# Yixin-F/DR-Using-SCV-OD

Measured on AMD Instinct MI355X. Metric: scans/sec on SemanticKITTI-seq-05-shaped input (SCV-OD dynamic-removal path, raw scans -> per-point labels + static map), higher is better.
Workload: dtype f32

## Files before the change

dr-using-scv-od_amd/csrc/scvod_k_patchwork.inc:

```
constexpr int kClsThreads = 256;
constexpr int kClsItems = 8;

__global__ __launch_bounds__(kClsThreads) void k_pw_classify(DevParams P, Arena A) {
    __shared__ int hist[kMaxPatches];
    const int s = blockIdx.y;
    const int base = A.scan_off[s];
    const int n = A.scan_off[s + 1] - base;
    const int start = blockIdx.x * (kClsThreads * kClsItems);
    if (start >= n) return;
    for (int b = threadIdx.x; b < P.n_patches; b += kClsThreads) hist[b] = 0;
    __syncthreads();
    float4 pt[kClsItems];
#pragma unroll
    for (int it = 0; it < kClsItems; ++it) {
        const int i = start + it * kClsThreads + threadIdx.x;
        pt[it] = A.pts[base + min(i, n - 1)];
    }
#pragma unroll
    for (int it = 0; it < kClsItems; ++it) {
        const int i = start + it * kClsThreads + threadIdx.x;
        if (i < n) {
            const float4 p = pt[it];
            int pid = czm_patch_of(P.czm, p.x, p.y, p.z);
            A.pid[base + i] = (int16_t)pid;
            A.zkey[base + i] = float_sort_key(p.z);
            if (pid >= 0) atomicAdd(&hist[pid], 1);
        }
    }
    __syncthreads();
    for (int b = threadIdx.x; b < P.n_patches; b += kClsThreads) {
        int c = hist[b];
        if (c) atomicAdd(&A.patch_count[s * kMaxPatches + b], c);
    }
}

__global__ __launch_bounds__(1024) void k_pw_offsets(DevParams P, Arena A) {
    __shared__ int wsum[17];
    const int s = blockIdx.x;
    int c = (threadIdx.x < (unsigned)P.n_patches) ? A.patch_count[s * kMaxPatches + threadIdx.x] : 0;
    int total;
    int ex = block_excl_scan<1024>(c, total, wsum);
    if (threadIdx.x <= (unsigned)P.n_patches) A.patch_off[s * (kMaxPatches + 1) + threadIdx.x] = ex;
}

__global__ __launch_bounds__(kClsThreads) void k_pw_scatter(DevParams P, Arena A) {
    __shared__ int hist[kMaxPatches];
    const int s = blockIdx.y;
    const int base = A.scan_off[s];
    const int n = A.scan_off[s + 1] - base;
    const int start = blockIdx.x * (kClsThreads * kClsItems);
    if (start >= n) return;
    for (int b = threadIdx.x; b < P.n_patches; b += kClsThreads) hist[b] = 0;
    __syncthreads();
    int pid[kClsItems], rank[kClsItems];
    uint32_t zk[kClsItems];
#pragma unroll
    for (int it = 0; it < kClsItems; ++it) {
        const int i = start + it * kClsThreads + threadIdx.x;
        pid[it] = (i < n) ? (int)A.pid[base + i] : -1;
        zk[it] = A.zkey[base + min(i, n - 1)];
    }
#pragma unroll
    for (int it = 0; it < kClsItems; ++it)
        rank[it] = wave_bin_rank(hist, pid[it]);
    __syncthreads();
    for (int b = threadIdx.x; b < P.n_patches; b += kClsThreads) {
        int c = hist[b];
        if (c) hist[b] = A.patch_off[s * (kMaxPatches + 1) + b] + atomicAdd(&A.patch_cursor[s * kMaxPatches + b], c);
    }
    __syncthreads();
#pragma unroll
    for (int it = 0; it < kClsItems; ++it) {
        int i = start + it * kClsThreads + threadIdx.x;
        if (i < n && pid[it] >= 0) A.keys[(size_t)base + hist[pid[it]] + rank[it]] = pack_key(zk[it], (uint32_t)i);
    }
}

constexpr int kClassXS = 32, kClassM = 40, kClassM2 = 44, kClassL = 48;
#ifndef SCVOD_FIT_COOP_CLASS
#define SCVOD_FIT_COOP_CLASS 36
#endif
constexpr int kClassFitCoop = SCVOD_FIT_COOP_CLASS;

__device__ __forceinline__ void order_range(const int32_t* off, int c_lo, int c_hi, int& lo, int& hi) {
    lo = off[c_hi];
    hi = (c_lo == 0) ? off[64] : off[c_lo - 1];
}

constexpr bool pw_sort_padfree(int cap) { return SCVOD_SORT_PADFREE == 2 || (SCVOD_SORT_PADFREE == 1 && cap >= 2048); }
constexpr bool pw_sort_merge(int cap) {
    return pw_sort_padfree(cap) && cap >= 2048 && cap <= 8192 && (SCVOD_SORT_MERGE == 2 || (SCVOD_SORT_MERGE == 1 && cap >= 4096));
}

template <int CAP, int THREADS, int C_LO, int C_HI, int LGE>
__global__ __launch_bounds__(THREADS)
__attribute__((amdgpu_waves_per_eu(pw_sort_padfree(CAP) ? (CAP >= 1024 ? 4 : 6) : 1, 8)))
void k_pw_sort(DevParams P, Arena A) {
    extern __shared__ __attribute__((aligned(16))) unsigned char smem[];
    int lo, hi;
    order_range(A.order_off, C_LO, C_HI, lo, hi);
    constexpr int PK = (CAP == 4096) ? 1 : 2;
    constexpr bool PADFREE = pw_sort_padfree(CAP);
    constexpr bool MERGE = pw_sort_merge(CAP) && LGE == 4 && (THREADS << LGE) == CAP;
    PROF_BEGIN();
    for (int w = lo + blockIdx.x; w < hi; w += gridDim.x) {
        const int4 item = A.order[w];
        const int n = item.y, base = item.z, off = item.w;
        const bool in_lds = (n <= CAP);
        unsigned long long* keys;
        if (CAP >= 4096) PROF_RESET();
        if (in_lds) {
            keys = (unsigned long long*)smem;
            int np2 = 1 << LGE;
            while (np2 < n) np2 <<= 1;
            const int nlive = sortnet::live_end(n, LGE);
            constexpr int IT = CAP / THREADS;
            const unsigned long long* gk = (const unsigned long long*)A.keys + (size_t)base + off;
            bool from_regs = false;
            if constexpr (IT == (1 << LGE) && CAP >= 4096) {
                if (np2 == CAP) {
                    from_regs = true;
                    unsigned long long tmp[IT];
                    if constexpr (PADFREE) {
                        if ((int)threadIdx.x < (nlive >> LGE)) {
#pragma unroll
                            for (int it = 0; it < IT; ++it) {
                                const int j = sortnet::start_key(it, (int)threadIdx.x, nlive, LGE);
                                tmp[it] = (j < n) ? gk[j] : kKeyPad;
                            }
                        }
                        if (CAP >= 4096) PROF_MARK(PK, 0);
                        if constexpr (MERGE)
                            mergepath_sort_regs<THREADS, true, LGE, SCVOD_SORT_MERGE_RUN>(tmp, keys, np2, nlive, (unsigned long long)kKeyPad);
                        else
                            padfree_sort_regs<THREADS, true, LGE>(tmp, keys, np2, nlive, (unsigned long long)kKeyPad);
                    } else {
#pragma unroll
                        for (int it = 0; it < IT; ++it) {
                            const int j = it * THREADS + (int)threadIdx.x;
                            tmp[it] = (j < n) ? gk[j] : kKeyPad;
                        }
                        if (CAP >= 4096) PROF_MARK(PK, 0);
                        block_bitonic_sort_pow2_regs<THREADS, true, LGE>(tmp, keys);
                    }
                }
            }
            if (!from_regs) {
                const int nfill = PADFREE ? nlive : np2;
                for (int j = threadIdx.x; j < nfill; j += THREADS) keys[sort_slot<true>(j)] = (j < n) ? gk[j] : kKeyPad;
                __syncthreads();
                if (CAP >= 4096) PROF_MARK(PK, 0);
                if constexpr (MERGE)
                    mergepath_sort<THREADS, true, LGE, SCVOD_SORT_MERGE_RUN>(keys, np2, nlive, (unsigned long long)kKeyPad);
                else if constexpr (PADFREE)
                    padfree_sort<THREADS, true, LGE>(keys, np2, nlive, (unsigned long long)kKeyPad);
                else
                    block_bitonic_sort_pow2<THREADS, true, LGE>(keys, np2);
            }
            if (CAP >= 4096) PROF_MARK(PK, 1);
        } else {
            keys = (unsigned long long*)(A.keys + (size_t)base + off);
            block_bitonic_sort<THREADS, false>(keys, n);
        }
        Xyz* dst = A.sorted_xyz + (size_t)base + off;
        uint32_t* dsti = A.sorted_idx + (size_t)base + off;
        for (int j0 = threadIdx.x; j0 < n; j0 += 4 * THREADS) {
            uint32_t id[4];
            float4 q[4];
#pragma unroll
            for (int u = 0; u < 4; ++u) {
                const int j = min(j0 + u * THREADS, n - 1);
                id[u] = key_idx(keys[in_lds ? sort_slot<true>(j) : j]);
            }
#pragma unroll
            for (int u = 0; u < 4; ++u) q[u] = A.pts[base + id[u]];
#pragma unroll
            for (int u = 0; u < 4; ++u) {
                const int j = j0 + u * THREADS;
                if (j < n) {
                    Xyz o;
                    o.x = q[u].x;
                    o.y = q[u].y;
                    o.z = q[u].z;
                    dst[j] = o;
                    dsti[j] = id[u];
                }
            }
        }
        __syncthreads();
        if (CAP >= 4096) PROF_MARK(PK, 2);
    }
}

constexpr int kClassWave = 24;
__global__ __launch_bounds__(256) void k_pw_sort_wave(DevParams P, Arena A) {
    const int lane = threadIdx.x & 63;
    const int wave = threadIdx.x >> 6;
    int lo, hi;
    order_range(A.order_off, 0, kClassWave - 1, lo, hi);
    for (int w = lo + blockIdx.x * 4 + wave; w < hi; w += gridDim.x * 4) {
        const int4 item = A.order[w];
        const int n = item.y, base = item.z, off = item.w;
        unsigned long long key = (lane < n) ? A.keys[(size_t)base + off + lane] : kKeyPad;
#pragma unroll
        for (int k = 2; k <= 64; k <<= 1) {
#pragma unroll
            for (int j = k >> 1; j >= 1; j >>= 1) {
                const unsigned long long other = __shfl_xor(key, j, 64);
                const bool take_min = (((lane & k) == 0) == ((lane & j) == 0));
                unsigned long long mn = key, mx = other;
                cswap_asc(mn, mx);
                key = take_min ? mn : mx;
            }
        }
        if (lane < n) {
            const uint32_t id = key_idx(key);
            const float4 q = A.pts[base + id];
            Xyz o;
            o.x = q.x;
            o.y = q.y;
            o.z = q.z;
            A.sorted_xyz[(size_t)base + off + lane] = o;
            A.sorted_idx[(size_t)base + off + lane] = id;
        }
    }
}

__device__ __forceinline__ int pw_size_class(int n) {
    int lg = 31 - __clz(n);
    int frac = (lg >= 2) ? ((n >> (lg - 2)) & 3) : 0;
    int c = lg * 4 + frac;
    return c > 63 ? 63 : c;
}

__global__ __launch_bounds__(256) void k_pw_order_count(DevParams P, Arena A) {
    __shared__ int hist[64];
    if (threadIdx.x < 64) hist[threadIdx.x] = 0;
    __syncthreads();
    const int t = blockIdx.x * 256 + threadIdx.x;
    if (t < A.n_scans * P.n_patches) {
        const int s = t / P.n_patches, p = t - s * P.n_patches;
        const int n = A.patch_count[s * kMaxPatches + p];
        if (n <= P.czm.num_min_pts) {
            PatchRec r = {n, 0, 0, 0, 0};
            A.patch_rec[s * kMaxPatches + p] = r;
            scvod_patch_plane pl = {};
            pl.n_pts = n;
            A.planes[s * kMaxPatches + p] = pl;
        } else {
            atomicAdd(&hist[pw_size_class(n)], 1);
        }
    }
    __syncthreads();
    if (threadIdx.x < 64 && hist[threadIdx.x]) atomicAdd(&A.order_hist[threadIdx.x], hist[threadIdx.x]);
}

__global__ __launch_bounds__(64) void k_pw_order_offsets(Arena A) {
    const int c = 63 - threadIdx.x;
    const int v = A.order_hist[c];
    const int inc = wave_incl_scan(v);
    A.order_off[c] = inc - v;
    if (threadIdx.x == 63) A.order_off[64] = inc;
}

__global__ __launch_bounds__(256) void k_pw_order_scatter(DevParams P, Arena A) {
    __shared__ int hist[64];
    if (threadIdx.x < 64) hist[threadIdx.x] = 0;
    __syncthreads();
    const int t = blockIdx.x * 256 + threadIdx.x;
    int c = -1, rank = 0;
    int4 item = make_int4(0, 0, 0, 0);
    if (t < A.n_scans * P.n_patches) {
        const int s = t / P.n_patches, p = t - s * P.n_patches;
        const int n = A.patch_count[s * kMaxPatches + p];
        if (n > P.czm.num_min_pts) {
            c = pw_size_class(n);
            rank = atomicAdd(&hist[c], 1);
            item = make_int4(s * kMaxPatches + p, n, A.scan_off[s], A.patch_off[s * (kMaxPatches + 1) + p]);
        }
    }
    __syncthreads();
    if (threadIdx.x < 64 && hist[threadIdx.x])
        hist[threadIdx.x] = A.order_off[threadIdx.x] + atomicAdd(&A.order_cursor[threadIdx.x], hist[threadIdx.x]);
    __syncthreads();
    if (c >= 0) A.order[hist[c] + rank] = item;
}

__global__ __launch_bounds__(256) void k_vx_order_count(DevParams P, Arena A) {
    __shared__ int hist[64];
    if (threadIdx.x < 64) hist[threadIdx.x] = 0;
    __syncthreads();
    const int t = blockIdx.x * 256 + threadIdx.x;
    if (t < A.n_scans * P.n_buckets) {
        const int s = t / P.n_buckets, b = t - s * P.n_buckets;
        const int m = A.vb_count[s * kMaxBuckets + b];
        if (m > 0)
            atomicAdd(&hist[pw_size_class(m)], 1);
        else
            A.vb_nvox[s * kMaxBuckets + b] = 0;
    }
    __syncthreads();
    if (threadIdx.x < 64 && hist[threadIdx.x]) atomicAdd(&A.vorder_hist[threadIdx.x], hist[threadIdx.x]);
}

__global__ __launch_bounds__(64) void k_vx_order_offsets(Arena A) {
    const int c = 63 - threadIdx.x;
    const int v = A.vorder_hist[c];
    const int inc = wave_incl_scan(v);
    A.vorder_off[c] = inc - v;
    if (threadIdx.x == 63) A.vorder_off[64] = inc;
}

__global__ __launch_bounds__(256) void k_vx_order_scatter(DevParams P, Arena A) {
    __shared__ int hist[64];
    if (threadIdx.x < 64) hist[threadIdx.x] = 0;
    __syncthreads();
    const int t = blockIdx.x * 256 + threadIdx.x;
    int c = -1, rank = 0;
    int4 item = make_int4(0, 0, 0, 0);
    if (t < A.n_scans * P.n_buckets) {
        const int s = t / P.n_buckets, b = t - s * P.n_buckets;
        const int m = A.vb_count[s * kMaxBuckets + b];
        if (m > 0) {
            c = pw_size_class(m);
            rank = atomicAdd(&hist[c], 1);
            item = make_int4(s * kMaxBuckets + b, m, A.scan_off[s], A.vb_off[s * (kMaxBuckets + 1) + b]);
        }
    }
    __syncthreads();
    if (threadIdx.x < 64 && hist[threadIdx.x])
        hist[threadIdx.x] = A.vorder_off[threadIdx.x] + atomicAdd(&A.vorder_cursor[threadIdx.x], hist[threadIdx.x]);
    __syncthreads();
    if (c >= 0) A.vorder[hist[c] + rank] = item;
}

__device__ __forceinline__ float plane_res(const Xyz& q, float n0, float n1, float n2) {
    float r = q.x * n0;
    r = r + q.y * n1;
    r = r + q.z * n2;
    return r;
}

struct FitState {
    float cov[9];
    float mean0, mean1, mean2;
    float n0, n1, n2, thd;
    float sv0, sv1, sv2;
};
__device__ __forceinline__ void fit_state_init(FitState& F) {
#pragma unroll
    for (int k = 0; k < 9; ++k) F.cov[k] = 0.f;
    F.mean0 = F.mean1 = F.mean2 = 0.f;
    F.n0 = F.n1 = F.n2 = F.thd = 0.f;
    F.sv0 = F.sv1 = F.sv2 = 0.f;
}

__device__ __forceinline__ void fit_update(FitState& F, const CzmParams& cz, float a0, float a1, float a2, float a3, float a4,
                                           float a5, float a6, float a7, float a8, int m) {
    if (m != 0) {
        const float fn = (float)m;
        a0 = a0 / fn;
        a1 = a1 / fn;
        a2 = a2 / fn;
        a3 = a3 / fn;
        a4 = a4 / fn;
        a5 = a5 / fn;
        a6 = a6 / fn;
        a7 = a7 / fn;
        a8 = a8 / fn;
        F.mean0 = a6;
        F.mean1 = a7;
        F.mean2 = a8;
        F.cov[0] = a0 - a6 * a6;
        F.cov[1] = a1 - a6 * a7;
        F.cov[2] = a2 - a6 * a8;
        F.cov[4] = a3 - a7 * a7;
        F.cov[5] = a4 - a7 * a8;
        F.cov[8] = a5 - a8 * a8;
        F.cov[3] = F.cov[1];
        F.cov[6] = F.cov[2];
        F.cov[7] = F.cov[5];
    }
    Svd3 sv;
    svd3_jacobi(F.cov, sv);
    F.n0 = sv.U[2];
    F.n1 = sv.U[5];
    F.n2 = sv.U[8];
    F.sv0 = sv.sv[0];
    F.sv1 = sv.sv[1];
    F.sv2 = sv.sv[2];
    float dot = F.n0 * F.mean0;
    dot = dot + F.n1 * F.mean1;
    dot = dot + F.n2 * F.mean2;
    const float d = -dot;
    F.thd = (float)(cz.th_dist - (double)d);
}

__device__ __forceinline__ int fit_status(const DevParams& P, int zone, int ring, int concentric_idx, const FitState& F) {
    const double ground_z_vec = (double)fabs_f(F.n2);
    const double ground_z_elevation = (double)F.mean2;
    float svmin = F.sv0;
    if (F.sv1 < svmin) svmin = F.sv1;
    if (F.sv2 < svmin) svmin = F.sv2;
    const double surface_variable = (double)(svmin / (F.sv0 + F.sv1 + F.sv2));
    if (ground_z_vec < P.czm.uprightness_thr) return 2;
    if (concentric_idx < P.czm.num_rings_of_interest) {
        const int e = ring + 2 * zone;
        if (ground_z_elevation > P.czm.elevation_thr[e]) return (P.czm.flatness_thr[e] > surface_variable) ? 1 : 3;
    }
    return 1;
}

__device__ __forceinline__ void fit_finish(const DevParams& P, const Arena& A, int s, int p, int n, int zone, int ring,
                                           int concentric_idx, const FitState& F) {
    const float n0 = F.n0, n1 = F.n1, n2 = F.n2, thd = F.thd, mean0 = F.mean0, mean1 = F.mean1, mean2 = F.mean2;
    const float sv0 = F.sv0, sv1 = F.sv1, sv2 = F.sv2;
    const int status = fit_status(P, zone, ring, concentric_idx, F);
    scvod_patch_plane pl;
    pl.normal[0] = n0;
    pl.normal[1] = n1;
    pl.normal[2] = n2;
    pl.mean[0] = mean0;
    pl.mean[1] = mean1;
    pl.mean[2] = mean2;
    pl.sv[0] = sv0;
    pl.sv[1] = sv1;
    pl.sv[2] = sv2;
    pl.n_pts = n;
    pl.n_ground = 0;
    pl.status = status;
    A.planes[s * kMaxPatches + p] = pl;
    A.fit_thd[s * kMaxPatches + p] = thd;
}

__device__ __forceinline__ uint32_t triple_of_point(const DevParams& P, float x, float y, float z) {
    int32_t ri, si, ai;
    if (!idx3_fast(P.bin, P.binfast, x, y, z, &ri, &si, &ai)) {
        Apri a;
// ... 725 lines not shown
```

dr-using-scv-od_amd/csrc/scvod_kernels.hip:

```cpp
#include <type_traits>

#include "scvod_boxgrid.h"
#include "scvod_grid.h"
#include "scvod_sortnet.h"
#include "scvod_mergepath.h"
#include <rocprim/device/device_radix_sort.hpp>

namespace scvod {

#ifdef SCVOD_PROFILE
__device__ unsigned long long g_prof[8][16];
#define PROF_BEGIN() unsigned long long t_prev = wall_clock64()
#define PROF_RESET()                                   \
    do {                                               \
        __syncthreads();                               \
        if (threadIdx.x == 0) t_prev = wall_clock64(); \
    } while (0)
#define PROF_MARK(k, i)                                      \
    do {                                                     \
        __syncthreads();                                     \
        if (threadIdx.x == 0) {                              \
            const unsigned long long t_now = wall_clock64(); \
            atomicAdd(&g_prof[k][i], t_now - t_prev);        \
            t_prev = t_now;                                  \
// ... 27 lines not shown
    const T INF = ~(T)0;
    int np2 = 8;
    while (np2 < n) np2 <<= 1;
    for (int g = threadIdx.x; g < (np2 >> 3); g += THREADS) {
        const int b = g << 3;
        if (b >= n) continue;
        T e[8];
#pragma unroll
        for (int m = 0; m < 8; ++m) e[m] = (b + m < n) ? a[IX(b + m)] : INF;
        cswap(e[0], e[1]); cswap(e[2], e[3]); cswap(e[4], e[5]); cswap(e[6], e[7]);
        cswap(e[0], e[2]); cswap(e[1], e[3]); cswap(e[4], e[6]); cswap(e[5], e[7]);
        cswap(e[1], e[2]); cswap(e[5], e[6]);
        cswap(e[0], e[4]); cswap(e[1], e[5]); cswap(e[2], e[6]); cswap(e[3], e[7]);
        cswap(e[2], e[4]); cswap(e[3], e[5]);
        cswap(e[1], e[2]); cswap(e[3], e[4]); cswap(e[5], e[6]);
#pragma unroll
        for (int m = 0; m < 8; ++m)
            if (b + m < n) a[IX(b + m)] = e[m];
    }
    __syncthreads();
    const int half = np2 >> 1;
    for (int k = 16; k <= np2; k <<= 1) {
        const int hk = k >> 1;
        for (int t = threadIdx.x; t < half; t += THREADS) {
            const int blk = t / hk, off = t - blk * hk;
            const int i = blk * k + off, j = blk * k + (k - 1 - off);
            if (j < n) {
                T x = a[IX(i)], y = a[IX(j)];
                if (x > y) {
                    a[IX(i)] = y;
                    a[IX(j)] = x;
                }
            }
        }
        __syncthreads();
        int j = k >> 2;
        while (j >= 1) {
            if (j >= 4) {
                const int jl = j >> 2;
                for (int t = threadIdx.x; t < (np2 >> 3); t += THREADS) {
                    const int b = (t / jl) * (jl << 3) + (t % jl);
                    if (b >= n) continue;
                    T e[8];
#pragma unroll
                    for (int m = 0; m < 8; ++m) e[m] = (b + m * jl < n) ? a[IX(b + m * jl)] : INF;
                    cswap(e[0], e[4]); cswap(e[1], e[5]); cswap(e[2], e[6]); cswap(e[3], e[7]);
                    cswap(e[0], e[2]); cswap(e[1], e[3]); cswap(e[4], e[6]); cswap(e[5], e[7]);
                    cswap(e[0], e[1]); cswap(e[2], e[3]); cswap(e[4], e[5]); cswap(e[6], e[7]);
#pragma unroll
                    for (int m = 0; m < 8; ++m)
                        if (b + m * jl < n) a[IX(b + m * jl)] = e[m];
                }
                j >>= 3;
            } else if (j == 2) {
                for (int t = threadIdx.x; t < (np2 >> 2); t += THREADS) {
                    const int b = t << 2;
                    if (b >= n) continue;
                    T e[4];
#pragma unroll
                    for (int m = 0; m < 4; ++m) e[m] = (b + m < n) ? a[IX(b + m)] : INF;
                    cswap(e[0], e[2]); cswap(e[1], e[3]);
                    cswap(e[0], e[1]); cswap(e[2], e[3]);
#pragma unroll
                    for (int m = 0; m < 4; ++m)
                        if (b + m < n) a[IX(b + m)] = e[m];
                }
                j = 0;
            } else {
                for (int t = threadIdx.x; t < half; t += THREADS) {
                    const int i = t << 1;
                    if (i + 1 < n) {
                        T x = a[IX(i)], y = a[IX(i + 1)];
                        if (x > y) {
                            a[IX(i)] = y;
                            a[IX(i + 1)] = x;
                        }
                    }
                }
                j = 0;
            }
            __syncthreads();
        }
    }
}
#undef IX

__device__ __forceinline__ int wave_bin_rank(int* hist, int bin) {
    const int lane = threadIdx.x & 63;
    int rank = 0;
    bool todo = bin >= 0;
    while (__any(todo)) {
        const int first = __ffsll((long long)__ballot(todo)) - 1;
        const int b0 = __shfl(bin, first);
        const bool mine = todo && (bin == b0);
        const unsigned long long mask = __ballot(mine);
        int old = 0;
        if (lane == first) old = atomicAdd(&hist[b0], __popcll(mask));
        old = __shfl(old, first);
        if (mine) {
            rank = old + __popcll(mask & ((1ull << lane) - 1ull));
            todo = false;
        }
    }
    return rank;
}
__device__ __forceinline__ void wave_bin_add(int* hist, int bin) {
    const int lane = threadIdx.x & 63;
    bool todo = bin >= 0;
    while (__any(todo)) {
        const int first = __ffsll((long long)__ballot(todo)) - 1;
        const int b0 = __shfl(bin, first);
        const bool mine = todo && (bin == b0);
        const unsigned long long mask = __ballot(mine);
        if (lane == first) atomicAdd(&hist[b0], __popcll(mask));
        if (mine) todo = false;
    }
}

constexpr int kKeyIdxBits = 19;
static_assert((1 << kKeyIdxBits) >= SCVOD_MAX_SCAN_POINTS, "index field of the sort keys");
constexpr unsigned long long kKeyExp = 0x3ffull << 52;
constexpr unsigned long long kKeyPad = 0x4000000000000000ull;
__device__ __forceinline__ unsigned long long pack_key(uint32_t key, uint32_t idx) {
    return kKeyExp | ((unsigned long long)key << kKeyIdxBits) | idx;
}
__device__ __forceinline__ uint32_t key_idx(unsigned long long k) { return (uint32_t)k & ((1u << kKeyIdxBits) - 1u); }
__device__ __forceinline__ uint32_t key_major(unsigned long long k) { return (uint32_t)(k >> kKeyIdxBits); }


__device__ __forceinline__ void cswap_asc(unsigned long long& x, unsigned long long& y) {
    double lo, hi;
    const double dx = __longlong_as_double((long long)x), dy = __longlong_as_double((long long)y);
    asm("v_min_f64 %0, %1, %2" : "=v"(lo) : "v"(dx), "v"(dy));
    asm("v_max_f64 %0, %1, %2" : "=v"(hi) : "v"(dx), "v"(dy));
    x = (unsigned long long)__double_as_longlong(lo);
    y = (unsigned long long)__double_as_longlong(hi);
}
__device__ __forceinline__ void cswap_asc(uint32_t& x, uint32_t& y) {
    const uint32_t lo = x < y ? x : y;
    const uint32_t hi = x < y ? y : x;
    x = lo;
    y = hi;
}

template <int LT, typename T>
__device__ __forceinline__ void reg_merge(T (&e)[1 << LT]) {
#pragma unroll
    for (int d = (1 << LT) >> 1; d >= 1; d >>= 1) {
#pragma unroll
        for (int m = 0; m < (1 << LT); ++m)
            if ((m & d) == 0) cswap_asc(e[m], e[m + d]);
    }
}

template <int THREADS, bool PAD, int LT, typename T>
__device__ __forceinline__ void bitonic_pass(T* a, int np2, int k, int r) {
    constexpr int E = 1 << LT;
    const int jl = 1 << (r - LT);
    for (int t = threadIdx.x; t < (np2 >> LT); t += THREADS) {
        const int b = ((t >> (r - LT)) << r) | (t & (jl - 1));
        const int rev = ((b & k) == 0) ? 0 : (E - 1);
        T e[E];
#pragma unroll
        for (int m = 0; m < E; ++m) e[m] = a[sort_slot<PAD>(b + (m ^ rev) * jl)];
        reg_merge<LT>(e);
#pragma unroll
        for (int m = 0; m < E; ++m) a[sort_slot<PAD>(b + (m ^ rev) * jl)] = e[m];
    }
    __syncthreads();
}

template <bool PAD, int LGE, typename T>
__device__ __forceinline__ void bitonic_run_to_lds(T (&e)[1 << LGE], T* a, int b) {
    constexpr int E = 1 << LGE;
#pragma unroll
    for (int kk = 2; kk <= E; kk <<= 1) {
#pragma unroll
        for (int d = kk >> 1; d >= 1; d >>= 1) {
#pragma unroll
            for (int m = 0; m < E; ++m)
                if ((m & d) == 0) {
                    if (kk == E || (m & kk) == 0)
                        cswap_asc(e[m], e[m + d]);
                    else
                        cswap_asc(e[m + d], e[m]);
                }
        }
    }
    const int rev = ((b & E) == 0) ? 0 : (E - 1);
#pragma unroll
    for (int m = 0; m < E; ++m) a[sort_slot<PAD>(b + (m ^ rev))] = e[m];
}

template <int THREADS, bool PAD, int LGE, typename T>
__device__ __forceinline__ void block_bitonic_merge_stages(T* a, int np2);

template <int THREADS, bool PAD, int LGE, typename T>
__device__ __forceinline__ void block_bitonic_sort_pow2(T* a, int np2) {
    constexpr int E = 1 << LGE;
    for (int g = threadIdx.x; g < (np2 >> LGE); g += THREADS) {
        const int b = g << LGE;
        T e[E];
#pragma unroll
        for (int m = 0; m < E; ++m) e[m] = a[sort_slot<PAD>(b + m)];
        bitonic_run_to_lds<PAD, LGE>(e, a, b);
    }
    __syncthreads();
    block_bitonic_merge_stages<THREADS, PAD, LGE>(a, np2);
}

template <int THREADS, bool PAD, int LGE, typename T>
__device__ __forceinline__ void block_bitonic_sort_pow2_regs(T (&e)[1 << LGE], T* a) {
    bitonic_run_to_lds<PAD, LGE>(e, a, (int)threadIdx.x << LGE);
    __syncthreads();
    block_bitonic_merge_stages<THREADS, PAD, LGE>(a, THREADS << LGE);
}

template <int THREADS, bool PAD, int LGE, typename T>
__device__ __forceinline__ void block_bitonic_merge_stages(T* a, int np2) {
    constexpr int E = 1 << LGE;
    int lgk = LGE + 1;
    for (int k = 2 * E; k <= np2; k <<= 1, ++lgk) {
        int r = lgk;
        const int first = (r % LGE) ? (r % LGE) : LGE;
        if (first == 1)
            bitonic_pass<THREADS, PAD, 1>(a, np2, k, r);
        else if (first == 2)
            bitonic_pass<THREADS, PAD, 2>(a, np2, k, r);
        else if (first == 3)
            bitonic_pass<THREADS, PAD, 3>(a, np2, k, r);
        else
            bitonic_pass<THREADS, PAD, 4>(a, np2, k, r);
        r -= first;
        while (r > 0) {
            bitonic_pass<THREADS, PAD, LGE>(a, np2, k, r);
            r -= LGE;
        }
    }
}

#ifndef SCVOD_SORT_PADFREE
#define SCVOD_SORT_PADFREE 1
#endif
#ifndef SCVOD_VOX_PADFREE
#define SCVOD_VOX_PADFREE 1
#endif
struct CxAsc {
    template <typename T>
    __device__ __forceinline__ void operator()(T& lo, T& hi) const { cswap_asc(lo, hi); }
};

template <int THREADS, bool PAD, int LT, bool MIRROR, typename T>
__device__ __forceinline__ void padfree_pass(T* a, int np2, int nlive, int r, T padv) {
    const int items = sortnet::pass_items(np2, nlive, r, LT);
    for (int t = threadIdx.x; t < items; t += THREADS) sortnet::pass_item<LT, MIRROR, PAD, T>(a, t, r, nlive, padv, CxAsc{});
    __syncthreads();
}

template <int THREADS, bool PAD, int LGE, typename T>
__device__ __forceinline__ void padfree_merge_stages(T* a, int np2, int nlive, T padv) {
    sortnet::for_each_pass<LGE>(np2, [&](int r, int lt, bool mirror) {
        if (!mirror)
            padfree_pass<THREADS, PAD, LGE, false>(a, np2, nlive, r, padv);
        else if (lt == 1)
            padfree_pass<THREADS, PAD, 1, true>(a, np2, nlive, r, padv);
        else if (lt == 2)
            padfree_pass<THREADS, PAD, 2, true>(a, np2, nlive, r, padv);
        else if (lt == 3 || LGE == 3)
            padfree_pass<THREADS, PAD, 3, true>(a, np2, nlive, r, padv);
        else if constexpr (LGE >= 4)
            padfree_pass<THREADS, PAD, 4, true>(a, np2, nlive, r, padv);
    });
}

template <int THREADS, bool PAD, int LGE, typename T>
__device__ __forceinline__ void padfree_sort(T* a, int np2, int nlive, T padv) {
    constexpr int E = 1 << LGE;
    for (int g = threadIdx.x; g < (nlive >> LGE); g += THREADS) {
        T e[E];
#pragma unroll
        for (int m = 0; m < E; ++m) e[m] = a[sort_slot<PAD>((g << LGE) + m)];
        sortnet::run_store<LGE, PAD>(e, a, g, CxAsc{});
    }
    __syncthreads();
    padfree_merge_stages<THREADS, PAD, LGE>(a, np2, nlive, padv);
}

template <int THREADS, bool PAD, int LGE, typename T>
__device__ __forceinline__ void padfree_sort_regs(T (&e)[1 << LGE], T* a, int np2, int nlive, T padv) {
    if ((int)threadIdx.x < (nlive >> LGE)) sortnet::run_store<LGE, PAD>(e, a, (int)threadIdx.x, CxAsc{});
    __syncthreads();
    padfree_merge_stages<THREADS, PAD, LGE>(a, np2, nlive, padv);
}

#ifndef SCVOD_SORT_MERGE
#define SCVOD_SORT_MERGE 1
#endif
#ifndef SCVOD_SORT_MERGE_RUN
#define SCVOD_SORT_MERGE_RUN 16
#endif
static_assert(SCVOD_SORT_MERGE_RUN >= 16 && SCVOD_SORT_MERGE_RUN <= 1024 && (SCVOD_SORT_MERGE_RUN & (SCVOD_SORT_MERGE_RUN - 1)) == 0,
              "SCVOD_SORT_MERGE_RUN");

template <int THREADS, bool PAD, int LGE, int RUN, typename T>
__device__ __forceinline__ void mergepath_levels(T* a, int np2, int nlive, T padv) {
    static_assert(RUN >= (1 << LGE), "the merge levels start from whole register runs");
    if constexpr (RUN > (1 << LGE)) {
        sortnet::for_each_pass<LGE>(np2 < RUN ? np2 : RUN, [&](int r, int lt, bool mirror) {
            if (!mirror)
                padfree_pass<THREADS, PAD, LGE, false>(a, np2, nlive, r, padv);
            else if (lt == 1)
                padfree_pass<THREADS, PAD, 1, true>(a, np2, nlive, r, padv);
            else if (lt == 2)
                padfree_pass<THREADS, PAD, 2, true>(a, np2, nlive, r, padv);
            else if (lt == 3 || LGE == 3)
                padfree_pass<THREADS, PAD, 3, true>(a, np2, nlive, r, padv);
            else if constexpr (LGE >= 4)
                padfree_pass<THREADS, PAD, 4, true>(a, np2, nlive, r, padv);
        });
    }
    for (int L = RUN; L < nlive; L <<= 1) {
        T out[1 << LGE];
        const bool mine = mergepath::merge_window<LGE, PAD, T>(a, (int)threadIdx.x, L, nlive, out, ~(T)0);
        __syncthreads();
        if (mine) mergepath::store_window<LGE, PAD, T>(a, (int)threadIdx.x, out);
        __syncthreads();
    }
}

template <int THREADS, bool PAD, int LGE, int RUN, typename T>
__device__ __forceinline__ void mergepath_sort(T* a, int np2, int nlive, T padv) {
    constexpr int E = 1 << LGE;
    for (int g = threadIdx.x; g < (nlive >> LGE); g += THREADS) {
        T e[E];
#pragma unroll
        for (int m = 0; m < E; ++m) e[m] = a[sort_slot<PAD>((g << LGE) + m)];
        sortnet::run_store<LGE, PAD>(e, a, g, CxAsc{});
    }
    __syncthreads();
    mergepath_levels<THREADS, PAD, LGE, RUN>(a, np2, nlive, padv);
}
template <int THREADS, bool PAD, int LGE, int RUN, typename T>
__device__ __forceinline__ void mergepath_sort_regs(T (&e)[1 << LGE], T* a, int np2, int nlive, T padv) {
    if ((int)threadIdx.x < (nlive >> LGE)) sortnet::run_store<LGE, PAD>(e, a, (int)threadIdx.x, CxAsc{});
    __syncthreads();
    mergepath_levels<THREADS, PAD, LGE, RUN>(a, np2, nlive, padv);
}

#include "scvod_k_patchwork.inc"
#include "scvod_k_voxelgrid.inc"
#include "scvod_k_voxels.inc"
#include "scvod_k_cluster.inc"
#include "scvod_k_merge.inc"
#include "scvod_k_rgrow.inc"
#include "scvod_k_calib.inc"
#include "scvod_k_probe_nn.inc"
#define TH_BEGIN(name) \
    if (th) th(tu, name, 1)
#define TH_END(name) \
    if (th) th(tu, name, 0)

#ifndef SCVOD_SORT_LGE
#define SCVOD_SORT_LGE 4
#endif
constexpr int kLGE = SCVOD_SORT_LGE;
constexpr int kTS = (kLGE == 4) ? 1 : 2;
#ifndef SCVOD_VOX_LGE
#define SCVOD_VOX_LGE 3
#endif
constexpr int kLGEv = SCVOD_VOX_LGE, kTSv = (kLGEv == 4) ? 1 : 2;
constexpr int kPersistCUs = 256;
constexpr int kSortCapS = 1024, kSortThreadsS = 64;
constexpr int kSortCapL = 8192, kSortThreadsL = 512;
constexpr int kSortCapXL = 16384, kClassXL = 52;
constexpr size_t sort_lds_bytes(int cap) { return (size_t)(cap + cap / 8) * 8; }
constexpr int kVoxCapS = 1024, kVoxThreadsS = 64;
constexpr int kVoxCapL = 8192, kVoxThreadsL = 512;

template <int CAP, int THREADS, int C_LO, int C_HI, int LGE, typename KT, bool DESC>
static void launch_vx_tier(const DevParams& P, const Arena& A, hipStream_t st, int per_cu_network) {
    if constexpr (vx_bucket_counting(CAP, sizeof(KT), 0, DESC)) {
        if (P.vb_shift == kVxCountShift) {
            constexpr size_t lds = vox_lds_bytes(CAP, sizeof(KT), DESC, true);
            constexpr int per_cu_counting = vx_count_per_cu(CAP, DESC);
            static_assert(per_cu_counting > 0 && per_cu_counting * lds <= 160 * 1024, "workgroups per CU of a counting tier");
            if (CAP >= 4096)
                hipFuncSetAttribute((const void*)k_vx_bucket<CAP, THREADS, C_LO, C_HI, LGE, 0, KT, DESC, true>, hipFuncAttributeMaxDynamicSharedMemorySize, (int)lds);
            hipLaunchKernelGGL((k_vx_bucket<CAP, THREADS, C_LO, C_HI, LGE, 0, KT, DESC, true>), dim3(kPersistCUs * per_cu_counting), dim3(THREADS), lds, st, P, A);
            return;
        }
    }
    constexpr size_t lds = vox_lds_bytes(CAP, sizeof(KT), DESC);
    if (CAP >= 4096)
        hipFuncSetAttribute((const void*)k_vx_bucket<CAP, THREADS, C_LO, C_HI, LGE, 0, KT, DESC, false>, hipFuncAttributeMaxDynamicSharedMemorySize, (int)lds);
    hipLaunchKernelGGL((k_vx_bucket<CAP, THREADS, C_LO, C_HI, LGE, 0, KT, DESC, false>), dim3(kPersistCUs * per_cu_network), dim3(THREADS), lds, st, P, A);
}

void launch_process(const DevParams& P, const Arena& A, hipStream_t st, int do_patchwork, int apply_filter,
                    int do_voxels, TimerHook th, void* tu, int lean_voxels, int lean_emit) {
    const int B = A.n_scans;
    if (B <= 0) return;
    if (do_patchwork == 1) {
        hipMemsetAsync(A.patch_count, 0, sizeof(int32_t) * (size_t)B * kMaxPatches, st);
        hipMemsetAsync(A.patch_cursor, 0, sizeof(int32_t) * (size_t)B * kMaxPatches, st);
        dim3 gcls((A.max_scan_pts + kClsThreads * kClsItems - 1) / (kClsThreads * kClsItems), B);
        TH_BEGIN("pw_classify");
        hipLaunchKernelGGL(k_pw_classify, gcls, dim3(kClsThreads), 0, st, P, A);
        TH_END("pw_classify");
        TH_BEGIN("pw_offsets");
        hipLaunchKernelGGL(k_pw_offsets, dim3(B), dim3(1024), 0, st, P, A);
        TH_END("pw_offsets");
        TH_BEGIN("pw_scatter");
        hipLaunchKernelGGL(k_pw_scatter, gcls, dim3(kClsThreads), 0, st, P, A);
        TH_END("pw_scatter");
        hipMemsetAsync(A.order_hist, 0, sizeof(int32_t) * 64, st);
        hipMemsetAsync(A.order_cursor, 0, sizeof(int32_t) * 64, st);
        const int n_all = B * P.n_patches;
        TH_BEGIN("pw_order");
        hipLaunchKernelGGL(k_pw_order_count, dim3((n_all + 255) / 256), dim3(256), 0, st, P, A);
        hipLaunchKernelGGL(k_pw_order_offsets, dim3(1), dim3(64), 0, st, A);
        hipLaunchKernelGGL(k_pw_order_scatter, dim3((n_all + 255) / 256), dim3(256), 0, st, P, A);
        TH_END("pw_order");
        hipFuncSetAttribute((const void*)k_pw_sort<kSortCapXL, 1024, kClassXL, 63, 4>, hipFuncAttributeMaxDynamicSharedMemorySize,
                            (int)sort_lds_bytes(kSortCapXL));
        hipFuncSetAttribute((const void*)k_pw_sort<kSortCapL, kSortThreadsL * kTS, kClassL, kClassXL - 1, kLGE>,
                            hipFuncAttributeMaxDynamicSharedMemorySize, (int)sort_lds_bytes(kSortCapL));
        TH_BEGIN("pw_sort_8192");
        hipLaunchKernelGGL((k_pw_sort<kSortCapXL, 1024, kClassXL, 63, 4>), dim3(kPersistCUs), dim3(1024), sort_lds_bytes(kSortCapXL), st, P, A);
        hipLaunchKernelGGL((k_pw_sort<kSortCapL, kSortThreadsL * kTS, kClassL, kClassXL - 1, kLGE>), dim3(kPersistCUs * 2),
                           dim3(kSortThreadsL * kTS), sort_lds_bytes(kSortCapL), st, P, A);
        TH_END("pw_sort_8192");
        TH_BEGIN("pw_sort_4096");
        hipLaunchKernelGGL((k_pw_sort<4096, 256 * kTS, kClassM2, kClassL - 1, kLGE>), dim3(kPersistCUs * 4), dim3(256 * kTS),
                           sort_lds_bytes(4096), st, P, A);
        TH_END("pw_sort_4096");
        TH_BEGIN("pw_sort_2048");
        hipLaunchKernelGGL((k_pw_sort<2048, 128 * kTS, kClassM, kClassM2 - 1, kLGE>), dim3(kPersistCUs * 8), dim3(128 * kTS),
                           sort_lds_bytes(2048), st, P, A);
        TH_END("pw_sort_2048");
        TH_BEGIN("pw_sort_1024");
        hipLaunchKernelGGL((k_pw_sort<kSortCapS, kSortThreadsS * kTS, kClassXS, kClassM - 1, kLGE>), dim3(kPersistCUs * 16),
                           dim3(kSortThreadsS * kTS), sort_lds_bytes(kSortCapS), st, P, A);
        TH_END("pw_sort_1024");
        TH_BEGIN("pw_sort_256");
        hipLaunchKernelGGL((k_pw_sort<256, 64, kClassWave, kClassXS - 1, 3>), dim3(kPersistCUs * 32), dim3(64),
                           sort_lds_bytes(256), st, P, A);
        TH_END("pw_sort_256");
        TH_BEGIN("pw_sort_wave");
        hipLaunchKernelGGL(k_pw_sort_wave, dim3(kPersistCUs * 8), dim3(256), 0, st, P, A);
        TH_END("pw_sort_wave");
        const int coop_class = (B <= 8) ? kClassWave : kClassFitCoop;
        const int coop_min = 1 << (coop_class / 4);
        TH_BEGIN("pw_fit_large");
        const dim3 gfit((int)(A.total_pts / coop_min / (B <= 8 ? 1 : 4)) + 1);
        if (B <= 8) {
            if (lean_emit)
                hipLaunchKernelGGL((k_pw_fit_coop<64, true>), gfit, dim3(64), 0, st, P, A, coop_class);
            else
                hipLaunchKernelGGL((k_pw_fit_coop<64, false>), gfit, dim3(64), 0, st, P, A, coop_class);
        } else {
            if (lean_emit)
                hipLaunchKernelGGL((k_pw_fit_coop<16, true>), gfit, dim3(64), 0, st, P, A, coop_class);
            else
                hipLaunchKernelGGL((k_pw_fit_coop<16, false>), gfit, dim3(64), 0, st, P, A, coop_class);
        }
        TH_END("pw_fit_large");
        TH_BEGIN("pw_fit");
        hipLaunchKernelGGL(k_pw_fit, dim3((n_all + 63) / 64), dim3(64), 0, st, P, A, coop_class);
        TH_END("pw_fit");
        TH_BEGIN("pw_arrange");
        if (lean_emit) {
            if (coop_class > kClassWave) hipLaunchKernelGGL((k_pw_arrange<64, true>), dim3(kPersistCUs * 8), dim3(256), 0, st, P, A, kClassWave, coop_class - 1);
            hipLaunchKernelGGL((k_pw_arrange<16, true>), dim3(kPersistCUs * 4), dim3(256), 0, st, P, A, 0, kClassWave - 1);
        } else {
            if (coop_class > kClassWave) hipLaunchKernelGGL((k_pw_arrange<64, false>), dim3(kPersistCUs * 8), dim3(256), 0, st, P, A, kClassWave, coop_class - 1);
            hipLaunchKernelGGL((k_pw_arrange<16, false>), dim3(kPersistCUs * 4), dim3(256), 0, st, P, A, 0, kClassWave - 1);
        }
        TH_END("pw_arrange");
        TH_BEGIN("emit_offsets");
        hipLaunchKernelGGL(k_emit_offsets, dim3(B), dim3(1024), 0, st, P, A);
        TH_END("emit_offsets");
        TH_BEGIN("emit");
        if (lean_emit)
            hipLaunchKernelGGL(k_emit<true>, dim3(kPersistCUs * 8), dim3(kEmitThreads), 0, st, P, A);
        else
            hipLaunchKernelGGL(k_emit<false>, dim3(kPersistCUs * 8), dim3(kEmitThreads), 0, st, P, A);
        TH_END("emit");
    } else if (do_patchwork == 0) {
        TH_BEGIN("bin_direct");
        hipLaunchKernelGGL(k_bin_direct, dim3(B), dim3(1024), 0, st, P, A, apply_filter);
        TH_END("bin_direct");
    }
    if (do_voxels) {
        if (do_patchwork == 2) {
            hipMemsetAsync(A.scan_irr, 0, sizeof(int32_t) * (size_t)B, st);
            hipMemsetAsync(A.irr_list, 0xff, sizeof(int32_t) * (size_t)B * (kIrrListCap + 1), st);
            hipLaunchKernelGGL(k_apri_split, dim3((A.max_scan_pts + 2047) / 2048, B), dim3(256), 0, st, A);
        }
        TH_BEGIN("vx_partition");
        hipLaunchKernelGGL(k_vx_partition, dim3(B), dim3(1024), 0, st, P, A);
        TH_END("vx_partition");
        dim3 gb(P.n_buckets, B);
        hipMemsetAsync(A.vorder_hist, 0, sizeof(int32_t) * 64, st);
        hipMemsetAsync(A.vorder_cursor, 0, sizeof(int32_t) * 64, st);
        const int nb_all = B * P.n_buckets;
        TH_BEGIN("vx_order");
        hipLaunchKernelGGL(k_vx_order_count, dim3((nb_all + 255) / 256), dim3(256), 0, st, P, A);
        hipLaunchKernelGGL(k_vx_order_offsets, dim3(1), dim3(64), 0, st, A);
        hipLaunchKernelGGL(k_vx_order_scatter, dim3((nb_all + 255) / 256), dim3(256), 0, st, P, A);
        TH_END("vx_order");
        if (do_patchwork == 3) {
            hipFuncSetAttribute((const void*)k_vx_bucket<kVoxCapL, kVoxThreadsL * kTSv, kClassL, 63, kLGEv, 1>,
                                hipFuncAttributeMaxDynamicSharedMemorySize, (int)vox_lds_bytes(kVoxCapL));
            hipFuncSetAttribute((const void*)k_vx_bucket<4096, 256 * kTSv, kClassM2, kClassL - 1, kLGEv, 1>,
                                hipFuncAttributeMaxDynamicSharedMemorySize, (int)vox_lds_bytes(4096));
            hipLaunchKernelGGL((k_vx_bucket<kVoxCapL, kVoxThreadsL * kTSv, kClassL, 63, kLGEv, 1>), dim3(kPersistCUs), dim3(kVoxThreadsL * kTSv),
                               vox_lds_bytes(kVoxCapL), st, P, A);
            hipLaunchKernelGGL((k_vx_bucket<4096, 256 * kTSv, kClassM2, kClassL - 1, kLGEv, 1>), dim3(kPersistCUs * 2), dim3(256 * kTSv),
                               vox_lds_bytes(4096), st, P, A);
            hipLaunchKernelGGL((k_vx_bucket<2048, 128 * kTSv, kClassM, kClassM2 - 1, kLGEv, 1>), dim3(kPersistCUs * 4), dim3(128 * kTSv),
                               vox_lds_bytes(2048), st, P, A);
            hipLaunchKernelGGL((k_vx_bucket<kVoxCapS, kVoxThreadsS * kTSv, kClassXS, kClassM - 1, kLGEv, 1>), dim3(kPersistCUs * 8),
                               dim3(kVoxThreadsS * kTSv), vox_lds_bytes(kVoxCapS), st, P, A);
            hipLaunchKernelGGL((k_vx_bucket<256, 64, 0, kClassXS - 1, 3, 1>), dim3(kPersistCUs * 32), dim3(64), vox_lds_bytes(256), st,
                               P, A);
            hipLaunchKernelGGL(k_vx_final_offsets, dim3(B), dim3(1024), 0, st, P, A);
            return;
        }
        auto bucket_tiers = [&](auto kt, auto desc) {
            using KT = decltype(kt);
            constexpr size_t KS = sizeof(KT);
            constexpr bool DESC = decltype(desc)::value;
            constexpr int kMore = (KS == 4 && SCVOD_VOX_K32_LDS) ? (DESC ? 3 : SCVOD_VOX_LEAN_MORE) : 2;
            TH_BEGIN("vx_bucket_8192");
            launch_vx_tier<kVoxCapL, kVoxThreadsL * kTSv, kClassL, 63, kLGEv, KT, DESC>(P, A, st, 1);
            TH_END("vx_bucket_8192");
            TH_BEGIN("vx_bucket_4096");
            launch_vx_tier<4096, 256 * kTSv, kClassM2, kClassL - 1, kLGEv, KT, DESC>(P, A, st, kMore);
            TH_END("vx_bucket_4096");
            TH_BEGIN("vx_bucket_2048");
            launch_vx_tier<2048, 128 * kTSv, kClassM, kClassM2 - 1, kLGEv, KT, DESC>(P, A, st, kMore * 2);
            TH_END("vx_bucket_2048");
            TH_BEGIN("vx_bucket_1024");
            launch_vx_tier<kVoxCapS, kVoxThreadsS * kTSv, kClassXS, kClassM - 1, kLGEv, KT, DESC>(P, A, st, DESC ? 8 : SCVOD_VOX_LEAN_S);
            TH_END("vx_bucket_1024");
            TH_BEGIN("vx_bucket_256");
            launch_vx_tier<256, 64, 0, kClassXS - 1, 3, KT, DESC>(P, A, st, 32);
            TH_END("vx_bucket_256");
        };
        if (A.vx_k32) {
            if (lean_voxels)
                bucket_tiers((uint32_t)0, std::false_type{});
            else
                bucket_tiers((uint32_t)0, std::true_type{});
        } else {
            if (lean_voxels)
                bucket_tiers((unsigned long long)0, std::false_type{});
            else
                bucket_tiers((unsigned long long)0, std::true_type{});
        }
        TH_BEGIN("vx_final_offsets");
        hipLaunchKernelGGL(k_vx_final_offsets, dim3(B), dim3(1024), 0, st, P, A);
        TH_END("vx_final_offsets");
        TH_BEGIN("vx_final");
        if (lean_voxels)
            hipLaunchKernelGGL(k_vx_final<false>, dim3((P.n_buckets + 3) / 4, B), dim3(256), 0, st, P, A);
        else
            hipLaunchKernelGGL(k_vx_final<true>, dim3((P.n_buckets + 3) / 4, B), dim3(256), 0, st, P, A);
        TH_END("vx_final");
    }
}

void launch_vox_descriptors(const Arena& A, int s0, int n_scans, hipStream_t st, TimerHook th, void* tu) {
    if (n_scans <= 0 || A.max_scan_pts <= 0) return;
    TH_BEGIN("vx_descriptors");
    hipLaunchKernelGGL(k_vx_descriptors, dim3((A.max_scan_pts + 4095) / 4096, n_scans), dim3(256), 0, st, A, s0);
    TH_END("vx_descriptors");
}

void launch_apri_intensity(const Arena& A, hipStream_t st, TimerHook th, void* tu) {
    if (A.n_scans <= 0 || A.max_scan_pts <= 0) return;
    TH_BEGIN("emit_intensity");
    hipLaunchKernelGGL(k_apri_intensity, dim3((A.max_scan_pts + 2047) / 2048, A.n_scans), dim3(256), 0, st, A);
    TH_END("emit_intensity");
}

void launch_emit_lists(const Arena& A, hipStream_t st, TimerHook th, void* tu) {
    if (A.n_scans <= 0 || A.max_scan_pts <= 0) return;
    TH_BEGIN("emit_lists");
    hipLaunchKernelGGL(k_emit_lists, dim3(kPersistCUs * 8), dim3(kEmitThreads), 0, st, A);
    TH_END("emit_lists");
}

void launch_apri_expand(const DevParams& P, const Arena& A, int s0, int n_scans, int max_pts, hipStream_t st) {
    if (n_scans <= 0 || max_pts <= 0) return;
    hipLaunchKernelGGL(k_apri_expand, dim3((max_pts + 1023) / 1024, n_scans), dim3(256), 0, st, P, A, s0);
}

void launch_voxelgrid_keys(const Arena& A, const VgJob& J, hipStream_t st) {
    const int B = A.n_scans;
    if (B <= 0) return;
    hipMemsetAsync(A.vg_range, 0, sizeof(int32_t), st);
    hipLaunchKernelGGL(k_vg_minmax, dim3(B), dim3(1024), 0, st, A, J);
    if (A.max_scan_pts > 0)
        hipLaunchKernelGGL(k_vg_keys, dim3((A.max_scan_pts + 2047) / 2048, B), dim3(256), 0, st, A, J);
}
void launch_voxelgrid_lut(const Arena& A, hipStream_t st) {
    if (A.n_scans <= 0 || A.max_scan_pts <= 0) return;
    hipFuncSetAttribute((const void*)k_vg_lut, hipFuncAttributeMaxDynamicSharedMemorySize, kVgLutBins * (int)sizeof(int));
    hipLaunchKernelGGL(k_vg_lut, dim3(A.n_scans), dim3(1024), kVgLutBins * sizeof(int), st, A, (int32_t*)A.vb_lut_shift);
}
void launch_voxelgrid_gather(const DevParams& P, const Arena& A, const VgJob& J, long long out_capacity, hipStream_t st) {
    if (A.n_scans <= 0 || A.max_scan_pts <= 0) return;
    hipLaunchKernelGGL(k_vg_outoff, dim3(1), dim3(1024), 0, st, A);
    hipLaunchKernelGGL(k_vg_final, dim3(P.n_buckets, A.n_scans), dim3(256), 0, st, A, J, out_capacity);
}

void launch_cls(const Arena& A, int s, size_t scan_base, int n_points, hipStream_t st) {
    if (n_points <= 0) return;
    hipMemsetAsync(A.cls + scan_base, SCVOD_CLS_DROPPED, (size_t)n_points, st);
    hipLaunchKernelGGL(k_cls_from_lists, dim3((n_points + 2047) / 2048), dim3(256), 0, st, A, s);
}

void launch_cluster(const DevParams& P, const Arena& A0, int from_apri, hipStream_t st, TimerHook th, void* tu) {
    Arena A = A0;
    hipMemsetAsync(A.cc_stats, 0, 8 * sizeof(int32_t), st);
    const int B = A.n_scans;
    if (B <= 0 || A.max_scan_pts <= 0) return;
    A.cc_help_blocks = A.cc_help_blocks_wanted > 0 ? 1 : 0;
    hipMemsetAsync(A.cc_again, 0, sizeof(int32_t), st);
    hipMemsetAsync(A.cc_help, 0, kCcHelpWords * sizeof(int32_t), st);
    hipFuncSetAttribute((const void*)k_cc_scan, hipFuncAttributeMaxDynamicSharedMemorySize, (int)kCcLdsBytes);
    hipFuncSetAttribute((const void*)k_cc_exact, hipFuncAttributeMaxDynamicSharedMemorySize, (int)kCcLdsBytes);
    TH_BEGIN("cc_scan");
    hipLaunchKernelGGL(k_cc_order, dim3(1), dim3(1024), 0, st, A);
    hipLaunchKernelGGL(k_cc_scan, dim3(B), dim3(kCcThreads), kCcLdsBytes, st, P, A, from_apri);
    TH_END("cc_scan");
    TH_BEGIN("cc_exact");
    hipLaunchKernelGGL(k_cc_exact, dim3(kCcExactBlocks), dim3(kCcThreads), kCcLdsBytes, st, P, A, from_apri);
    TH_END("cc_exact");
}

size_t merge_lds_bytes(const DevParams& P, int max_scan_pts) {
    return 4 * ((size_t)P.bin.range_num * P.bin.azimuth_num + 1 + ((size_t)max_scan_pts + 31) / 32);
}

void launch_merge(const DevParams& P, const Arena& A, const MergeJob& M, int from_apri, hipStream_t st, TimerHook th, void* tu) {
    hipMemsetAsync(M.stats, 0, 8 * sizeof(int32_t), st);
    const int B = A.n_scans;
// ... 197 lines not shown
```

dr-using-scv-od_amd/csrc/scvod_mergepath.h:

```cpp
#pragma once

#include "scvod_sortnet.h"

namespace mergepath {

struct Pair {
    int a0, a1;
    int b0, b1;
    int d;
};
SORTNET_HD constexpr int imin(int x, int y) { return x < y ? x : y; }
SORTNET_HD constexpr int imax(int x, int y) { return x > y ? x : y; }

SORTNET_HD constexpr Pair pair_of(int p, int L, int nlive) {
    const int a0 = p & ~(2 * L - 1);
    const int b0 = imin(a0 + L, nlive);
    return Pair{a0, b0, b0, imin(a0 + 2 * L, nlive), p - a0};
}

SORTNET_HD constexpr int levels(int run0, int nlive) {
    int c = 0;
    for (int L = run0; L < nlive; L <<= 1) ++c;
    return c;
}

template <bool PAD, typename T, typename Arr>
SORTNET_HD int split(Arr a, const Pair& q) {
    int lo = imax(0, q.d - (q.b1 - q.b0)), hi = imin(q.d, q.a1 - q.a0);
    while (lo < hi) {
        const int mid = (lo + hi) >> 1;
        const T ka = a[sortnet::slot(PAD, q.a0 + mid)];
        const T kb = a[sortnet::slot(PAD, q.b0 + q.d - 1 - mid)];
        if (kb < ka)
            hi = mid;
        else
            lo = mid + 1;
    }
    return lo;
}

template <int LGE, bool PAD, typename T, typename Arr>
SORTNET_HD bool merge_window(Arr a, int t, int L, int nlive, T (&out)[1 << LGE], T sent, int* ia = nullptr) {
    constexpr int E = 1 << LGE;
    const int p = t << LGE;
    if (p >= nlive) return false;
    const Pair q = pair_of(p, L, nlive);
    if (q.b0 == q.b1) return false;
    const int i = split<PAD, T>(a, q);
    if (ia) *ia = i;
    int xa = q.a0 + i, xb = q.b0 + (q.d - i);
    T ha = sent, hb = sent;
    if (xa < q.a1) ha = a[sortnet::slot(PAD, xa)];
    if (xb < q.b1) hb = a[sortnet::slot(PAD, xb)];
#pragma unroll
    for (int s = 0; s < E; ++s) {
        const bool take_a = !(hb < ha);
        out[s] = take_a ? ha : hb;
        if (s + 1 < E) {
            if (take_a) ++xa; else ++xb;
            const int x = take_a ? xa : xb;
            T v = sent;
            if (x < (take_a ? q.a1 : q.b1)) v = a[sortnet::slot(PAD, x)];
            if (take_a) ha = v; else hb = v;
        }
    }
    return true;
}

template <int LGE, bool PAD, typename T, typename Arr>
SORTNET_HD void store_window(Arr a, int t, const T (&out)[1 << LGE]) {
#pragma unroll
    for (int m = 0; m < (1 << LGE); ++m) a[sortnet::slot(PAD, (t << LGE) + m)] = out[m];
}

}
```

Measured before the change: 98420.

## Merge the first two sort levels in registers via DPP lane exchanges

Replaces the first two merge-path levels (runs of 16 to 64) with in-register bitonic-style merges between neighbouring lanes, using DPP quad permutes to exchange 64-bit keys. This avoids the LDS round trips, binary-search splits and barriers those levels needed. It also makes the merge path load keys into registers for every thread, padding lanes without a run, so whole quads take part. The cost is extra register pressure and compare-exchange ALU work, and the quad-lane mapping has to stay aligned with run boundaries.

Measured after the change: 99320 (median of 6 runs). About the same (+0.9%).

```diff
diff --git a/dr-using-scv-od_amd/csrc/scvod_k_patchwork.inc b/dr-using-scv-od_amd/csrc/scvod_k_patchwork.inc
--- a/dr-using-scv-od_amd/csrc/scvod_k_patchwork.inc
+++ b/dr-using-scv-od_amd/csrc/scvod_k_patchwork.inc
@@ -117,7 +117,20 @@
             constexpr int IT = CAP / THREADS;
             const unsigned long long* gk = (const unsigned long long*)A.keys + (size_t)base + off;
             bool from_regs = false;
-            if constexpr (IT == (1 << LGE) && CAP >= 4096) {
+            if constexpr (MERGE && CAP >= 4096) {
+                if (np2 == CAP) {
+                    from_regs = true;
+                    unsigned long long tmp[IT];
+                    const bool has_run = (int)threadIdx.x < (nlive >> LGE);
+#pragma unroll
+                    for (int it = 0; it < IT; ++it) {
+                        const int j = sortnet::start_key(it, (int)threadIdx.x, nlive, LGE);
+                        tmp[it] = (has_run && j < n) ? gk[j] : kKeyPad;
+                    }
+                    if (CAP >= 4096) PROF_MARK(PK, 0);
+                    mergepath_sort_regs<THREADS, true, LGE, SCVOD_SORT_MERGE_RUN>(tmp, keys, np2, nlive, (unsigned long long)kKeyPad);
+                }
+            } else if constexpr (IT == (1 << LGE) && CAP >= 4096) {
                 if (np2 == CAP) {
                     from_regs = true;
                     unsigned long long tmp[IT];
@@ -130,10 +143,7 @@
                             }
                         }
                         if (CAP >= 4096) PROF_MARK(PK, 0);
-                        if constexpr (MERGE)
-                            mergepath_sort_regs<THREADS, true, LGE, SCVOD_SORT_MERGE_RUN>(tmp, keys, np2, nlive, (unsigned long long)kKeyPad);
-                        else
-                            padfree_sort_regs<THREADS, true, LGE>(tmp, keys, np2, nlive, (unsigned long long)kKeyPad);
+                        padfree_sort_regs<THREADS, true, LGE>(tmp, keys, np2, nlive, (unsigned long long)kKeyPad);
                     } else {
 #pragma unroll
                         for (int it = 0; it < IT; ++it) {
diff --git a/dr-using-scv-od_amd/csrc/scvod_kernels.hip b/dr-using-scv-od_amd/csrc/scvod_kernels.hip
--- a/dr-using-scv-od_amd/csrc/scvod_kernels.hip
+++ b/dr-using-scv-od_amd/csrc/scvod_kernels.hip
@@ -353,9 +353,16 @@
 static_assert(SCVOD_SORT_MERGE_RUN >= 16 && SCVOD_SORT_MERGE_RUN <= 1024 && (SCVOD_SORT_MERGE_RUN & (SCVOD_SORT_MERGE_RUN - 1)) == 0,
               "SCVOD_SORT_MERGE_RUN");
 
-template <int THREADS, bool PAD, int LGE, int RUN, typename T>
+#ifndef SCVOD_SORT_LANEPAIR
+#define SCVOD_SORT_LANEPAIR 2
+#endif
+constexpr int kSortLaneLevels = SCVOD_SORT_MERGE_RUN == 16 ? SCVOD_SORT_LANEPAIR : 0;
+static_assert(kSortLaneLevels >= 0 && kSortLaneLevels <= 2, "SCVOD_SORT_LANEPAIR");
+
+template <int THREADS, bool PAD, int LGE, int RUN, int LANE_LEVELS, typename T>
 __device__ __forceinline__ void mergepath_levels(T* a, int np2, int nlive, T padv) {
     static_assert(RUN >= (1 << LGE), "the merge levels start from whole register runs");
+    static_assert(LANE_LEVELS == 0 || RUN == (1 << LGE), "the lane steps merge register runs");
     if constexpr (RUN > (1 << LGE)) {
         sortnet::for_each_pass<LGE>(np2 < RUN ? np2 : RUN, [&](int r, int lt, bool mirror) {
             if (!mirror)
@@ -370,7 +377,7 @@
                 padfree_pass<THREADS, PAD, 4, true>(a, np2, nlive, r, padv);
         });
     }
-    for (int L = RUN; L < nlive; L <<= 1) {
+    for (int L = RUN << LANE_LEVELS; L < nlive; L <<= 1) {
         T out[1 << LGE];
         const bool mine = mergepath::merge_window<LGE, PAD, T>(a, (int)threadIdx.x, L, nlive, out, ~(T)0);
         __syncthreads();
@@ -379,23 +386,61 @@
     }
 }
 
+template <int LGE, int QUAD_PERM>
+__device__ __forceinline__ void lane_fetch(const unsigned long long (&e)[1 << LGE], unsigned long long (&b)[1 << LGE]) {
+#pragma unroll
+    for (int m = 0; m < (1 << LGE); ++m) {
+        const int lo = __builtin_amdgcn_mov_dpp((int)(uint32_t)e[m], QUAD_PERM, 0xF, 0xF, false);
+        const int hi = __builtin_amdgcn_mov_dpp((int)(uint32_t)(e[m] >> 32), QUAD_PERM, 0xF, 0xF, false);
+        b[m] = ((unsigned long long)(uint32_t)hi << 32) | (uint32_t)lo;
+    }
+}
+template <int LGE>
+__device__ __forceinline__ void lanepair_step(unsigned long long (&e)[1 << LGE]) {
+    unsigned long long b[1 << LGE];
+    lane_fetch<LGE, 0xB1>(e, b);
+    mergepath::lanepair_merge<LGE>(e, b, (threadIdx.x & 1) != 0, CxAsc{});
+}
+template <int LGE>
+__device__ __forceinline__ void lanequad_step(unsigned long long (&e)[1 << LGE]) {
+    unsigned long long b[1 << LGE];
+    lane_fetch<LGE, 0x1B>(e, b);
+    mergepath::lanequad_merge_first<LGE>(e, b, (threadIdx.x & 2) != 0, CxAsc{});
+    lane_fetch<LGE, 0xB1>(e, b);
+    mergepath::lanequad_merge_second<LGE>(e, b, (threadIdx.x & 1) != 0, CxAsc{});
+}
+
+template <int THREADS, bool PAD, int LGE, int RUN, typename T>
+__device__ __forceinline__ void mergepath_runs(T (&e)[1 << LGE], T* a, bool has_run) {
+    if constexpr (kSortLaneLevels > 0 && RUN == (1 << LGE)) {
+        sortnet::run_network<LGE>(e, CxAsc{});
+        lanepair_step<LGE>(e);
+        if constexpr (kSortLaneLevels > 1) lanequad_step<LGE>(e);
+        if (has_run) {
+#pragma unroll
+            for (int m = 0; m < (1 << LGE); ++m) a[sort_slot<PAD>(((int)threadIdx.x << LGE) + m)] = e[m];
+        }
+    } else {
+        if (has_run) sortnet::run_store<LGE, PAD>(e, a, (int)threadIdx.x, CxAsc{});
+    }
+}
+
 template <int THREADS, bool PAD, int LGE, int RUN, typename T>
 __device__ __forceinline__ void mergepath_sort(T* a, int np2, int nlive, T padv) {
     constexpr int E = 1 << LGE;
-    for (int g = threadIdx.x; g < (nlive >> LGE); g += THREADS) {
-        T e[E];
-#pragma unroll
-        for (int m = 0; m < E; ++m) e[m] = a[sort_slot<PAD>((g << LGE) + m)];
-        sortnet::run_store<LGE, PAD>(e, a, g, CxAsc{});
-    }
+    const bool has_run = (int)threadIdx.x < (nlive >> LGE);
+    T e[E];
+#pragma unroll
+    for (int m = 0; m < E; ++m) e[m] = has_run ? a[sort_slot<PAD>(((int)threadIdx.x << LGE) + m)] : padv;
+    mergepath_runs<THREADS, PAD, LGE, RUN>(e, a, has_run);
     __syncthreads();
-    mergepath_levels<THREADS, PAD, LGE, RUN>(a, np2, nlive, padv);
+    mergepath_levels<THREADS, PAD, LGE, RUN, RUN == E ? kSortLaneLevels : 0>(a, np2, nlive, padv);
 }
 template <int THREADS, bool PAD, int LGE, int RUN, typename T>
 __device__ __forceinline__ void mergepath_sort_regs(T (&e)[1 << LGE], T* a, int np2, int nlive, T padv) {
-    if ((int)threadIdx.x < (nlive >> LGE)) sortnet::run_store<LGE, PAD>(e, a, (int)threadIdx.x, CxAsc{});
+    mergepath_runs<THREADS, PAD, LGE, RUN>(e, a, (int)threadIdx.x < (nlive >> LGE));
     __syncthreads();
-    mergepath_levels<THREADS, PAD, LGE, RUN>(a, np2, nlive, padv);
+    mergepath_levels<THREADS, PAD, LGE, RUN, RUN == (1 << LGE) ? kSortLaneLevels : 0>(a, np2, nlive, padv);
 }
 
 #include "scvod_k_patchwork.inc"
diff --git a/dr-using-scv-od_amd/csrc/scvod_mergepath.h b/dr-using-scv-od_amd/csrc/scvod_mergepath.h
--- a/dr-using-scv-od_amd/csrc/scvod_mergepath.h
+++ b/dr-using-scv-od_amd/csrc/scvod_mergepath.h
@@ -67,6 +67,40 @@
     return true;
 }
 
+template <int LGE, typename T, typename CX>
+SORTNET_HD void lane_mirror(T (&a)[1 << LGE], const T (&b)[1 << LGE], bool upper, CX cx) {
+    constexpr int E = 1 << LGE;
+#pragma unroll
+    for (int i = 0; i < E; ++i) {
+        T lo = a[i], hi = b[E - 1 - i];
+        cx(lo, hi);
+        a[i] = upper ? hi : lo;
+    }
+}
+template <int LGE, typename T, typename CX>
+SORTNET_HD void lane_butterfly(T (&a)[1 << LGE], const T (&b)[1 << LGE], bool upper, CX cx) {
+#pragma unroll
+    for (int i = 0; i < (1 << LGE); ++i) {
+        T lo = a[i], hi = b[i];
+        cx(lo, hi);
+        a[i] = upper ? hi : lo;
+    }
+}
+template <int LGE, typename T, typename CX>
+SORTNET_HD void lanepair_merge(T (&a)[1 << LGE], const T (&b)[1 << LGE], bool upper, CX cx) {
+    lane_mirror<LGE>(a, b, upper, cx);
+    sortnet::pass_network<LGE, false>(a, cx);
+}
+template <int LGE, typename T, typename CX>
+SORTNET_HD void lanequad_merge_first(T (&a)[1 << LGE], const T (&b)[1 << LGE], bool upper, CX cx) {
+    lane_mirror<LGE>(a, b, upper, cx);
+}
+template <int LGE, typename T, typename CX>
+SORTNET_HD void lanequad_merge_second(T (&a)[1 << LGE], const T (&b)[1 << LGE], bool upper, CX cx) {
+    lane_butterfly<LGE>(a, b, upper, cx);
+    sortnet::pass_network<LGE, false>(a, cx);
+}
+
 template <int LGE, bool PAD, typename T, typename Arr>
 SORTNET_HD void store_window(Arr a, int t, const T (&out)[1 << LGE]) {
 #pragma unroll
```
